# HSoumi/hybrid-als-twotower-recommender

Hardware: AMD Instinct MI355X
Metric: ALS epochs/sec + scored user-item pairs/sec at rank=64, 1/2/4/8 MI355X (higher is better)
Workload: dtype f64

## Files before the change

hybrid-als-twotower-recommender_amd/csrc/als_row.h:

```cpp
#pragma once
#include <type_traits>

#include "common.h"

#ifndef HREC_ALS_WAVES
#define HREC_ALS_WAVES 2
#endif
#ifndef HREC_ALS_CH0
#define HREC_ALS_CH0 8
#endif
#ifndef HREC_ALS_ABLATE
#define HREC_ALS_ABLATE 0
#endif
#ifndef HREC_ALS_SOLVE_UNROLL
#define HREC_ALS_SOLVE_UNROLL 8
#endif
#ifndef HREC_ALS_CH1
#define HREC_ALS_CH1 4
#endif
#ifndef HREC_ALS_PF
#define HREC_ALS_PF 8
#endif
#ifndef HREC_ALS_PF64
#define HREC_ALS_PF64 4
#endif
#ifndef HREC_ALS_ROT1DPP
#define HREC_ALS_ROT1DPP 1
#endif
#ifndef HREC_ALS_ROT1DPP64
#define HREC_ALS_ROT1DPP64 0
#endif
#ifndef HREC_ALS_PR
#define HREC_ALS_PR 2
#endif
#ifndef HREC_ALS_POOL_PF
#define HREC_ALS_POOL_PF 8
#endif
#ifndef HREC_ALS_POOL_PF64
#define HREC_ALS_POOL_PF64 4
#endif
#ifndef HREC_ALS_POOL_ROT1DPP64
#define HREC_ALS_POOL_ROT1DPP64 1
#endif

namespace hrec {

typedef double d4 __attribute__((ext_vector_type(4)));
typedef hrec_f4 f4;

template <int NT>
struct Vec;
template <>
struct Vec<4> {
  float x[4];
  __device__ static Vec load(const float* p) {
    const float4 t = *reinterpret_cast<const float4*>(p);
    return Vec{{t.x, t.y, t.z, t.w}};
  }
};
template <>
struct Vec<2> {
  float x[2];
  __device__ static Vec load(const float* p) {
    const float2 t = *reinterpret_cast<const float2*>(p);
    return Vec{{t.x, t.y}};
  }
};
template <>
struct Vec<1> {
  float x[1];
  __device__ static Vec load(const float* p) { return Vec{{*p}}; }
};

__device__ __forceinline__ int tri(int i) { return (i * (i + 1)) >> 1; }

typedef hrec_rsrc_t i4v;
typedef hrec_f2 f2;

struct VecD {
  double x[4];
};
__device__ __forceinline__ VecD struct_load_d(i4v rsrc, int vindex, int voffset) {
  const f4 lo = sbuf_load_f4(rsrc, vindex, voffset, 0, 0);
  const f4 hi = sbuf_load_f4(rsrc, vindex, voffset + 16, 0, 0);
  VecD v;
  v.x[0] = __hiloint2double(__float_as_int(lo.y), __float_as_int(lo.x));
  v.x[1] = __hiloint2double(__float_as_int(lo.w), __float_as_int(lo.z));
  v.x[2] = __hiloint2double(__float_as_int(hi.y), __float_as_int(hi.x));
  v.x[3] = __hiloint2double(__float_as_int(hi.w), __float_as_int(hi.z));
  return v;
}

struct VecD2 {
  double x[2];
};
__device__ __forceinline__ VecD2 struct_load_d2(i4v rsrc, int vindex, int voffset) {
  const f4 t = sbuf_load_f4(rsrc, vindex, voffset, 0, 0);
  VecD2 v;
  v.x[0] = __hiloint2double(__float_as_int(t.y), __float_as_int(t.x));
  v.x[1] = __hiloint2double(__float_as_int(t.w), __float_as_int(t.z));
  return v;
}

template <int NT>
__device__ __forceinline__ Vec<NT> struct_load(i4v rsrc, int vindex, int voffset) {
  Vec<NT> v;
  if constexpr (NT == 4) {
    const f4 t = sbuf_load_f4(rsrc, vindex, voffset, 0, 0);
    v.x[0] = t.x, v.x[1] = t.y, v.x[2] = t.z, v.x[3] = t.w;
  } else if constexpr (NT == 2) {
    const f2 t = sbuf_load_f2(rsrc, vindex, voffset, 0, 0);
    v.x[0] = t.x, v.x[1] = t.y;
  } else {
    v.x[0] = sbuf_load_f1(rsrc, vindex, voffset, 0, 0);
  }
  return v;
}

#ifdef HREC_ALS_STAMPS
__device__ unsigned long long g_als_stamps[8];
#define STAMP(i)                                                                      \
  do {                                                                                \
    __builtin_amdgcn_sched_barrier(0);                                                \
    const unsigned long long _t = __builtin_amdgcn_s_memtime();                       \
    __builtin_amdgcn_sched_barrier(0);                                                \
    if (threadIdx.x == 0 && (i) > 0) atomicAdd(&g_als_stamps[(i) > 0 ? (i) - 1 : 0], _t - _stamp_prev); \
    _stamp_prev = _t;                                                                 \
  } while (0)
#define STAMP_DECL unsigned long long _stamp_prev = 0
#else
#define STAMP(i) \
  do {           \
  } while (0)
#define STAMP_DECL
#endif

template <int N>
__device__ __forceinline__ double row_ror(double x) {
  const long long v = __double_as_longlong(x);
  const int lo = __builtin_amdgcn_mov_dpp((int)v, 0x120 + N, 0xf, 0xf, false);
  const int hi = __builtin_amdgcn_mov_dpp((int)(v >> 32), 0x120 + N, 0xf, 0xf, false);
  return __longlong_as_double(((long long)hi << 32) | (long long)(unsigned)lo);
}

__device__ __forceinline__ double bcast(double v, int src) {
  const long long x = __double_as_longlong(v);
  const int lo = __builtin_amdgcn_readlane((int)x, src);
  const int hi = __builtin_amdgcn_readlane((int)(x >> 32), src);
  return __longlong_as_double(((long long)hi << 32) | (long long)(unsigned)lo);
}

__device__ __forceinline__ void wave_lds_sync() {
  __builtin_amdgcn_fence(__ATOMIC_RELEASE, "wavefront");
  __builtin_amdgcn_wave_barrier();
  __builtin_amdgcn_fence(__ATOMIC_ACQUIRE, "wavefront");
}

template <int KP>
struct RowLds {
  static constexpr int kUp = KP * (KP + 1) / 2;
  static constexpr int kUpPad = ((kUp > 256 ? kUp : 256) + 1) & ~1;
  static constexpr int kSize = kUpPad + 128 + 3 * KP;
};

struct NoAcquire {};

template <int NT, int CH, int MODE, bool S64 = false, bool IMP = false, bool POOLED = false,
          typename Acq = NoAcquire>
__device__ __forceinline__ void gram_row(int64_t beg, int64_t end, int lane, const int32_t* __restrict__ indices,
                                         const float* __restrict__ values, const float* __restrict__ src,
                                         int64_t n_src, int k, double reg, d4 (&acc)[NT * (NT + 1) / 2],
                                         double* __restrict__ bsh, double* __restrict__ stage, double alpha = 0.0,
                                         const double* __restrict__ yty = nullptr, int* npos = nullptr,
                                         Acq acquire = Acq()) {
  constexpr bool kAcq = !std::is_same_v<Acq, NoAcquire>;
  static_assert(!kAcq || (NT == 4 && !IMP), "late slice acquisition: the kp-64 ring pipeline only");
  static_assert(!IMP || (MODE == 0 && !S64), "implicit feedback: f64 accumulation of f32 sources only");
  constexpr int KP = 16 * NT;
  constexpr int NPAIR = NT * (NT + 1) / 2;
  constexpr int CHN = 4 * CH;
  const int sub = lane >> 4;
  const int col = lane & 15;
  const int64_t n = end - beg;
  int n_pos = 0;

  STAMP_DECL;
  STAMP(0);
#pragma unroll
  for (int p = 0; p < NPAIR; ++p) acc[p] = d4{0.0, 0.0, 0.0, 0.0};
  if constexpr (HREC_ALS_ABLATE == 4) {
#pragma unroll
    for (int I = 0, p = 0; I < NT; p += NT - I, ++I)
#pragma unroll
      for (int rr = 0; rr < 4; ++rr) acc[p][rr] = (sub + 4 * rr == col) ? 1.0 + reg * (double)n : 0.0;
    if constexpr (kAcq) bsh = acquire() + RowLds<KP>::kUpPad + 128 + 2 * KP;
    if (lane < KP) bsh[lane] = 1.0;
    wave_lds_sync();
    return;
  }
  f4 fa[NPAIR];
  double bp[NT];
#pragma unroll
  for (int t = 0; t < NT; ++t) bp[t] = 0.0;

  auto load_iv = [&](int64_t base, int& ii, float& vv) {
    const int64_t p = base + (lane % CHN);
    const bool ok = (lane < CHN) && (p < end);
    ii = ok ? indices[p] : -1;
    vv = ok ? values[p] : 0.f;
  };
  auto gather = [&](Vec<NT> (&buf)[CH], int ii) {
#pragma unroll
    for (int s = 0; s < CH; ++s) {
      const int idx = __shfl(ii, 4 * s + sub, kWave);
      const int safe = idx < 0 ? 0 : idx;
      Vec<NT> v = Vec<NT>::load(src + (int64_t)safe * KP + NT * col);
#pragma unroll
      for (int t = 0; t < NT; ++t) v.x[t] = idx < 0 ? 0.f : v.x[t];
      buf[s] = v;
    }
  };

  if constexpr (NT == 4 && !IMP) {
  constexpr int PF = POOLED ? (S64 ? HREC_ALS_POOL_PF64 : HREC_ALS_POOL_PF) : (S64 ? HREC_ALS_PF64 : HREC_ALS_PF);
  static_assert(16 % PF == 0, "prefetch distance must divide the window");
  static_assert(!S64 || MODE == 0, "f64 sources: kp 64, f64 accumulation only");
  const int voff = (S64 ? 8 : 4) * NT * col;
  const int bp_addr = 4 * sub;
  const uint64_t sbase = (uint64_t)src;
  i4v rsrc;
  rsrc.x = __builtin_amdgcn_readfirstlane((int)(uint32_t)sbase);
  rsrc.y = __builtin_amdgcn_readfirstlane((int)(uint32_t)(sbase >> 32) | ((KP * (S64 ? 8 : 4)) << 16));
  rsrc.z = __builtin_amdgcn_readfirstlane((int)n_src);
  rsrc.w = 0x00020000;
  auto load_win = [&](int64_t w, int& ii, float& vv) {
    const int64_t p = beg + 64 * w + lane;
    const int64_t pc = p < end ? p : end - 1;
    const int iraw = indices[pc];
    const float vraw = values[pc];
    ii = p < end ? iraw : -1;
    vv = p < end ? vraw : 0.f;
  };
  auto bperm = [&](int win, int s) -> int { return __builtin_amdgcn_ds_bpermute(bp_addr + 16 * s, win); };
  const int64_t nsteps = (n + 3) >> 2;
  int iw0, iw1;
  float rw0, rw1;
  load_win(0, iw0, rw0);
  load_win(1, iw1, rw1);
  using RingT = std::conditional_t<S64, VecD, Vec<NT>>;
  auto ring_load = [&](int vi) -> RingT {
    if constexpr (S64) return struct_load_d(rsrc, vi, voff);
    else return struct_load<NT>(rsrc, vi, voff);
  };
  RingT ring[PF];
#pragma unroll
  for (int s = 0; s < PF; ++s) ring[s] = ring_load(bperm(iw0, s));
  int nidx = bperm(iw0, PF);
  constexpr bool kDiag4 = MODE == 0;
  constexpr int PR = HREC_ALS_PR;
  constexpr bool kRot1Dpp = S64 ? (POOLED ? HREC_ALS_POOL_ROT1DPP64 : HREC_ALS_ROT1DPP64) : HREC_ALS_ROT1DPP;
  static_assert(PR < PF, "rotated loads are issued from the current windows");
  const int voff1 = (S64 ? 8 : 4) * NT * ((col + 4) & 15), voff2 = (S64 ? 8 : 4) * NT * ((col + 8) & 15);
  auto rot_load = [&](int vi, int vo) -> RingT {
    if constexpr (S64) return struct_load_d(rsrc, vi, vo);
    else return struct_load<NT>(rsrc, vi, vo);
  };
  using PairT = std::conditional_t<S64, VecD2, Vec<2>>;
  const int hoff = (lane & 8) ? (S64 ? 16 : 8) : 0;
  auto pair_load = [&](int vi, int vo) -> PairT {
    if constexpr (S64) return struct_load_d2(rsrc, vi, vo);
    else return struct_load<2>(rsrc, vi, vo);
  };
  RingT rot1[PR];
  PairT rotA[PR], rotB[PR];
  if constexpr (kDiag4) {
#pragma unroll
    for (int q = 0; q < PR; ++q) {
      const int vi = bperm(iw0, q);
      if constexpr (!kRot1Dpp) rot1[q] = rot_load(vi, voff1);
      rotA[q] = pair_load(vi, voff + hoff);
      rotB[q] = pair_load(vi, voff2 + hoff);
    }
  }
  double dg[NT][3], dc[2];
#pragma unroll
  for (int t = 0; t < NT; ++t) dg[t][0] = dg[t][1] = 0.0;
#pragma unroll
  for (int t = 0; t < 2; ++t) dc[t] = 0.0;
  for (int64_t w = 0;; ++w) {
    int iw2;
    float rw2;
    load_win(w + 2, iw2, rw2);
    bool stop = false;
    const int rem = __builtin_amdgcn_readfirstlane((int)(nsteps - 16 * w < 16 ? nsteps - 16 * w : 16));
#pragma unroll
    for (int s = 0; s < 16; ++s) {
      if (s >= rem) {
        stop = true;
        break;
      }
      const RingT cur = ring[s % PF];
      double a[NT], ar1[NT], ar2[NT], apair[2];
#pragma unroll
      for (int t = 0; t < NT; ++t) a[t] = (double)cur.x[t];
      ring[s % PF] = ring_load(nidx);
      if constexpr (kDiag4) {
#pragma unroll
        for (int t = 0; t < NT; ++t) ar1[t] = kRot1Dpp ? row_ror<12>(a[t]) : (double)rot1[s % PR].x[t];
#pragma unroll
        for (int t = 0; t < 2; ++t) {
          apair[t] = (double)rotA[s % PR].x[t];
          ar2[t] = (double)rotB[s % PR].x[t];
        }
        const int vr = (s + PR < 16) ? bperm(iw0, s + PR) : bperm(iw1, s + PR - 16);
        if constexpr (!kRot1Dpp) rot1[s % PR] = rot_load(vr, voff1);
        rotA[s % PR] = pair_load(vr, voff + hoff);
        rotB[s % PR] = pair_load(vr, voff2 + hoff);
      }
      nidx = (s + 1 + PF < 16) ? bperm(iw0, s + 1 + PF) : bperm(iw1, s + 1 + PF - 16);
      const float rf = __int_as_float(__builtin_amdgcn_ds_bpermute(bp_addr + 16 * s, __float_as_int(rw0)));
      const double rv = (double)rf;
      if (MODE == 1 && (s % HREC_ALS_CH1) == 0) {
#pragma unroll
        for (int p = 0; p < NPAIR; ++p) fa[p] = f4{0.f, 0.f, 0.f, 0.f};
      }
      int p = 0;
#pragma unroll
      for (int I = 0; I < NT; ++I) {
#pragma unroll
        for (int J = I; J < NT; ++J) {
          if (MODE == 0) {
            if (I == J) {
              dg[I][0] = __builtin_amdgcn_mfma_f64_4x4x4f64(a[I], a[I], dg[I][0], 0, 0, 0);
              dg[I][1] = __builtin_amdgcn_mfma_f64_4x4x4f64(a[I], ar1[I], dg[I][1], 0, 0, 0);
              if (I < 2) dc[I] = __builtin_amdgcn_mfma_f64_4x4x4f64(apair[I], ar2[I], dc[I], 0, 0, 0);
            } else {
              acc[p] = __builtin_amdgcn_mfma_f64_16x16x4f64(a[I], a[J], acc[p], 0, 0, 0);
            }
          } else {
            fa[p] = __builtin_amdgcn_mfma_f32_16x16x4f32(cur.x[I], cur.x[J], fa[p], 0, 0, 0);
          }
          ++p;
        }
      }
#pragma unroll
      for (int t = 0; t < NT; ++t) bp[t] = fma(rv, a[t], bp[t]);
      if (MODE == 1 && ((s % HREC_ALS_CH1) == HREC_ALS_CH1 - 1 || s + 1 == rem)) {
#pragma unroll
        for (int p2 = 0; p2 < NPAIR; ++p2) {
#pragma unroll
          for (int rr = 0; rr < 4; ++rr) acc[p2][rr] += (double)fa[p2][rr];
        }
      }
    }
    if (stop || 16 * (w + 1) >= nsteps) break;
    iw0 = iw1;
    rw0 = rw1;
    iw1 = iw2;
    rw1 = rw2;
  }
  if constexpr (kAcq) {
    double* base = acquire();
    stage = base;
    bsh = base + RowLds<KP>::kUpPad + 128 + 2 * KP;
  }
  if constexpr (kDiag4) {
    const int i4 = lane >> 4, q4 = (lane >> 2) & 3, j4 = lane & 3;
#pragma unroll
    for (int I = 0, p = 0; I < NT; p += NT - I, ++I) {
#pragma unroll
      for (int sh = 0; sh < 3; ++sh) {
        const int r = 4 * q4 + i4, c = 4 * ((q4 + sh) & 3) + j4;
        if (sh == 2) {
          const bool mine = (q4 >= 2) == (I >= 2);
          const double v = dc[I & 1];
          stage[mine ? r * 16 + c : 256] = v;
          stage[mine ? c * 16 + r : 257] = v;
          continue;
        }
        stage[r * 16 + c] = dg[I][sh];
        stage[c * 16 + r] = dg[I][sh];
      }
      wave_lds_sync();
#pragma unroll
      for (int rr = 0; rr < 4; ++rr) acc[p][rr] = stage[(sub + 4 * rr) * 16 + col];
      wave_lds_sync();
    }
  }
  } else {
  int i0, i1;
  float r0, r1;
  load_iv(beg, i0, r0);
  load_iv(beg + CHN, i1, r1);
  Vec<NT> buf[CH];
  gather(buf, i0);

  for (int64_t base = beg; base < end; base += CHN) {
    Vec<NT> nbuf[CH];
    const bool more = base + CHN < end;
    if (more) gather(nbuf, i1);
    int i2;
    float r2;
    load_iv(base + 2 * CHN, i2, r2);
    if constexpr (IMP) n_pos += __builtin_popcountll(__ballot(r0 > 0.f));
    if (MODE == 1) {
#pragma unroll
      for (int p = 0; p < NPAIR; ++p) fa[p] = f4{0.f, 0.f, 0.f, 0.f};
    }
#pragma unroll
    for (int s = 0; s < CH; ++s) {
      const double rv = (double)__shfl(r0, 4 * s + sub, kWave);
      double a[NT];
#pragma unroll
      for (int t = 0; t < NT; ++t) a[t] = (double)buf[s].x[t];
      double aw[NT], bw = rv;
      if constexpr (IMP) {
        const double c1 = alpha * fabs(rv);
        bw = rv > 0.0 ? 1.0 + c1 : 0.0;
#pragma unroll
        for (int t = 0; t < NT; ++t) aw[t] = c1 * a[t];
      }
      auto lhs = [&](int t) -> double {
        if constexpr (IMP) return aw[t];
        else return a[t];
      };
      int p = 0;
#pragma unroll
      for (int I = 0; I < NT; ++I) {
#pragma unroll
        for (int J = I; J < NT; ++J) {
          if (MODE == 0)
            acc[p] = __builtin_amdgcn_mfma_f64_16x16x4f64(lhs(I), a[J], acc[p], 0, 0, 0);
          else
            fa[p] = __builtin_amdgcn_mfma_f32_16x16x4f32(buf[s].x[I], buf[s].x[J], fa[p], 0, 0, 0);
          ++p;
        }
      }
#pragma unroll
      for (int t = 0; t < NT; ++t) bp[t] = fma(bw, a[t], bp[t]);
    }
    if (MODE == 1) {
#pragma unroll
      for (int p = 0; p < NPAIR; ++p) {
#pragma unroll
        for (int rr = 0; rr < 4; ++rr) acc[p][rr] += (double)fa[p][rr];
      }
    }
    if (more) {
#pragma unroll
      for (int s = 0; s < CH; ++s) buf[s] = nbuf[s];
    }
    i0 = i1;
    r0 = r1;
    i1 = i2;
    r1 = r2;
  }
  }

  STAMP(1);
#pragma unroll
  for (int t = 0; t < NT; ++t) {
    bp[t] += __shfl_xor(bp[t], 16, kWave);
    bp[t] += __shfl_xor(bp[t], 32, kWave);
  }
  if (sub == 0) {
#pragma unroll
    for (int t = 0; t < NT; ++t) bsh[16 * t + col] = bp[t];
  }
  if (MODE == 1) {
#pragma unroll
    for (int p = 0; p < NPAIR; ++p) {
#pragma unroll
      for (int rr = 0; rr < 4; ++rr) stage[(4 * sub + rr) * 16 + col] = acc[p][rr];
      wave_lds_sync();
#pragma unroll
      for (int rr = 0; rr < 4; ++rr) acc[p][rr] = stage[(sub + 4 * rr) * 16 + col];
      wave_lds_sync();
    }
  }
  STAMP(2);
  if constexpr (IMP) {
    int p = 0;
#pragma unroll
    for (int I = 0; I < NT; ++I) {
#pragma unroll
      for (int J = I; J < NT; ++J) {
#pragma unroll
        for (int rr = 0; rr < 4; ++rr) acc[p][rr] += yty[(NT * (sub + 4 * rr) + I) * KP + NT * col + J];
        ++p;
      }
    }
    *npos = n_pos;
  }
  const double lambda = (double)(IMP ? (int64_t)n_pos : n) * reg;
  {
    int p = 0;
#pragma unroll
    for (int I = 0; I < NT; ++I) {
#pragma unroll
      for (int rr = 0; rr < 4; ++rr) {
        if (sub + 4 * rr == col) acc[p][rr] += (NT * col + I < k) ? lambda : 1.0;
      }
      p += NT - I;
    }
  }
}

template <int NT, bool LDSG>
__device__ __forceinline__ void factor_row_impl(int lane, d4 (&acc)[NT * (NT + 1) / 2], double* __restrict__ Up,
                                           double* __restrict__ scratch, const double* __restrict__ bsh,
                                           float* __restrict__ out) {
  constexpr int KP = 16 * NT;
  constexpr int NPAIR = NT * (NT + 1) / 2;
  double* __restrict__ colbuf = scratch;
  double* __restrict__ dsh = colbuf + 128;
  double* __restrict__ rdsh = dsh + KP;
  const int sub = lane >> 4, col = lane & 15;
  STAMP_DECL;
  STAMP(0);
  if constexpr (HREC_ALS_ABLATE == 1) {
    double sum = 0.0;
#pragma unroll
    for (int p = 0; p < NPAIR; ++p) sum += acc[p][0] + acc[p][1] + acc[p][2] + acc[p][3];
    wave_lds_sync();
    if (lane < KP) out[lane] = (float)(sum + bsh[lane]);
    return;
  }
  auto pidx = [](int I, int K) { return I * NT - (I * (I - 1)) / 2 + (K - I); };
  double bs = 0.0;
#pragma unroll
  for (int J = 0; J < NT; ++J) {
    if (!LDSG || J == 0) {
#pragma unroll
      for (int I = J; I < (LDSG ? NT : J + 1); ++I) {
#pragma unroll
        for (int K = I; K < NT; ++K) {
#pragma unroll
          for (int rr = 0; rr < 4; ++rr) {
            const int q = 16 * I + sub + 4 * rr, c = 16 * K + col;
            if (q <= c) Up[tri(c) + q] = acc[pidx(I, K)][rr];
          }
        }
      }
      wave_lds_sync();
    }
    if (J == 0) bs = lane < KP ? bsh[lane] : 0.0;
    const int c = lane;
    const bool own = c >= 16 * J && c < KP;
    double a[16];
#pragma unroll
    for (int m = 0; m < 16; ++m) {
      const int q = 16 * J + m;
      a[m] = (own && q <= c) ? Up[tri(c) + q] : 0.0;
    }
    double piv = bcast(a[0], 16 * J);
#pragma unroll
    for (int i = 0; i < 16; ++i) {
      const int pv = 16 * J + i;
      double* cb = colbuf + 64 * (i & 1);
      if (c < KP) cb[c] = a[i];
      const double r0 = __builtin_amdgcn_rcp(piv);
      const double r = fma(r0, fma(-piv, r0, 1.0), r0);
      const double ut = a[i] * r;
      if (own && c > pv) Up[tri(c) + pv] = ut;
      if (c == pv) {
        dsh[pv] = piv;
        rdsh[pv] = r;
      }
      {
        const double wq = bcast(bs, pv);
        if (own && c > pv) bs = fma(-ut, wq, bs);
      }
      if (i < 15) {
        piv = bcast(fma(-a[i], ut, a[i + 1]), pv + 1);
        wave_lds_sync();
#pragma unroll
        for (int m0 = (i + 1) & ~1; m0 < 16; m0 += 2) {
          const double2 u = *reinterpret_cast<const double2*>(cb + 16 * J + m0);
          if (m0 > i) a[m0] = fma(-u.x, ut, a[m0]);
          a[m0 + 1] = fma(-u.y, ut, a[m0 + 1]);
        }
      }
    }
    wave_lds_sync();
    if (J + 1 < NT) {
      double dq[4];
#pragma unroll
      for (int rr = 0; rr < 4; ++rr) dq[rr] = dsh[16 * J + sub + 4 * rr];
      d4 yv[NT];
#pragma unroll
      for (int K = J + 1; K < NT; ++K) {
#pragma unroll
        for (int rr = 0; rr < 4; ++rr) {
          const double x = Up[tri(16 * K + col) + 16 * J + sub + 4 * rr];
          acc[pidx(J, K)][rr] = x;
          yv[K][rr] = x * dq[rr];
        }
      }
#pragma unroll
      for (int K = J + 1; K < NT; ++K) {
#pragma unroll
        for (int M = K; M < NT; ++M) {
          if constexpr (LDSG) {
            d4 t;
#pragma unroll
            for (int rr = 0; rr < 4; ++rr) t[rr] = Up[tri(16 * M + col) + 16 * K + sub + 4 * rr];
#pragma unroll
            for (int rr = 0; rr < 4; ++rr)
              t = __builtin_amdgcn_mfma_f64_16x16x4f64(-acc[pidx(J, K)][rr], yv[M][rr], t, 0, 0, 0);
#pragma unroll
            for (int rr = 0; rr < 4; ++rr) {
              const int q = 16 * K + sub + 4 * rr, c = 16 * M + col;
              if (q <= c) Up[tri(c) + q] = t[rr];
            }
          } else {
#pragma unroll
            for (int rr = 0; rr < 4; ++rr)
              acc[pidx(K, M)] = __builtin_amdgcn_mfma_f64_16x16x4f64(-acc[pidx(J, K)][rr], yv[M][rr],
                                                                      acc[pidx(K, M)], 0, 0, 0);
          }
        }
      }
      if constexpr (LDSG) wave_lds_sync();
    }
  }
  STAMP(3);
  const int lc = lane < KP ? lane : KP - 1;
  const double myrd = rdsh[lc];
  if constexpr (HREC_ALS_ABLATE == 3) {
    if (lane < KP) out[lane] = (float)(myrd + Up[tri(lane)]);
    return;
  }
  double bi = bs * myrd;
#pragma unroll HREC_ALS_SOLVE_UNROLL
  for (int q = KP - 1; q >= 0; --q) {
    const double u = Up[tri(q) + (lane < KP ? lane : 0)];
    const double xq = bcast(bi, q);
    if (lane < q) bi = fma(-u, xq, bi);
  }
  STAMP(4);
  if (lane < KP) out[NT * (lane & 15) + (lane >> 4)] = (float)bi;
  wave_lds_sync();
}

template <int NT>
__device__ __forceinline__ void factor_row(int lane, d4 (&acc)[NT * (NT + 1) / 2], double* __restrict__ Up,
                                           double* __restrict__ scratch, const double* __restrict__ bsh,
                                           float* __restrict__ out) {
  factor_row_impl<NT, false>(lane, acc, Up, scratch, bsh, out);
}

template <int NT>
__device__ __forceinline__ void factor_row_lds(int lane, d4 (&acc)[NT * (NT + 1) / 2], double* __restrict__ Up,
                                               double* __restrict__ scratch, const double* __restrict__ bsh,
                                               float* __restrict__ out) {
  factor_row_impl<NT, true>(lane, acc, Up, scratch, bsh, out);
}

}
```

Measured before the change: 13.12.

## Block the in-panel Cholesky factorization into 4-column groups with MFMA trailing updates

Splits each 16-column panel factorization into groups of four columns. Scalar elimination runs only inside a group. The trailing update of the remaining sub-rows is done with f64 4x4x4 MFMA instructions on the accumulator registers, then written back to LDS. The goal is fewer per-lane scalar FMAs and smaller per-lane register arrays in the ALS normal-equation solve. In exchange it adds extra LDS round trips and barriers per group, and the accumulator layout now depends on MFMA semantics, which raises correctness risk.

```diff
diff --git a/hybrid-als-twotower-recommender_amd/csrc/als_row.h b/hybrid-als-twotower-recommender_amd/csrc/als_row.h
--- a/hybrid-als-twotower-recommender_amd/csrc/als_row.h
+++ b/hybrid-als-twotower-recommender_amd/csrc/als_row.h
@@ -512,6 +512,7 @@
                                            float* __restrict__ out) {
   constexpr int KP = 16 * NT;
   constexpr int NPAIR = NT * (NT + 1) / 2;
+  constexpr int G = 4;
   double* __restrict__ colbuf = scratch;
   double* __restrict__ dsh = colbuf + 128;
   double* __restrict__ rdsh = dsh + KP;
@@ -530,59 +531,91 @@
   double bs = 0.0;
 #pragma unroll
   for (int J = 0; J < NT; ++J) {
-    if (!LDSG || J == 0) {
-#pragma unroll
-      for (int I = J; I < (LDSG ? NT : J + 1); ++I) {
-#pragma unroll
-        for (int K = I; K < NT; ++K) {
-#pragma unroll
-          for (int rr = 0; rr < 4; ++rr) {
-            const int q = 16 * I + sub + 4 * rr, c = 16 * K + col;
-            if (q <= c) Up[tri(c) + q] = acc[pidx(I, K)][rr];
+    if constexpr (LDSG) {
+      if (J == 0) {
+#pragma unroll
+        for (int I = 0; I < NT; ++I) {
+#pragma unroll
+          for (int K = I; K < NT; ++K) {
+#pragma unroll
+            for (int rr = 0; rr < 4; ++rr) {
+              const int q = 16 * I + sub + 4 * rr, c = 16 * K + col;
+              if (q <= c) Up[tri(c) + q] = acc[pidx(I, K)][rr];
+            }
           }
         }
+        wave_lds_sync();
+      } else {
+#pragma unroll
+        for (int K = J; K < NT; ++K) {
+#pragma unroll
+          for (int rr = 1; rr < 4; ++rr) acc[pidx(J, K)][rr] = Up[tri(16 * K + col) + 16 * J + sub + 4 * rr];
+        }
+      }
+    } else {
+#pragma unroll
+      for (int K = J; K < NT; ++K) {
+        const int q = 16 * J + sub, c = 16 * K + col;
+        if (q <= c) Up[tri(c) + q] = acc[pidx(J, K)][0];
       }
       wave_lds_sync();
     }
     if (J == 0) bs = lane < KP ? bsh[lane] : 0.0;
     const int c = lane;
     const bool own = c >= 16 * J && c < KP;
-    double a[16];
-#pragma unroll
-    for (int m = 0; m < 16; ++m) {
-      const int q = 16 * J + m;
-      a[m] = (own && q <= c) ? Up[tri(c) + q] : 0.0;
-    }
-    double piv = bcast(a[0], 16 * J);
-#pragma unroll
-    for (int i = 0; i < 16; ++i) {
-      const int pv = 16 * J + i;
-      double* cb = colbuf + 64 * (i & 1);
-      if (c < KP) cb[c] = a[i];
-      const double r0 = __builtin_amdgcn_rcp(piv);
-      const double r = fma(r0, fma(-piv, r0, 1.0), r0);
-      const double ut = a[i] * r;
-      if (own && c > pv) Up[tri(c) + pv] = ut;
-      if (c == pv) {
-        dsh[pv] = piv;
-        rdsh[pv] = r;
-      }
-      {
-        const double wq = bcast(bs, pv);
-        if (own && c > pv) bs = fma(-ut, wq, bs);
-      }
-      if (i < 15) {
-        piv = bcast(fma(-a[i], ut, a[i + 1]), pv + 1);
+#pragma unroll
+    for (int g = 0; g < 16 / G; ++g) {
+      double a[G];
+#pragma unroll
+      for (int m = 0; m < G; ++m) {
+        const int q = 16 * J + G * g + m;
+        a[m] = (own && q <= c) ? Up[tri(c) + q] : 0.0;
+      }
+      double piv = bcast(a[0], 16 * J + G * g);
+#pragma unroll
+      for (int ii = 0; ii < G; ++ii) {
+        const int pv = 16 * J + G * g + ii;
+        double* cb = colbuf + 16 * ii;
+        if ((c >> 4) == J) cb[c & 15] = a[ii];
+        const double r0 = __builtin_amdgcn_rcp(piv);
+        const double r = fma(r0, fma(-piv, r0, 1.0), r0);
+        const double ut = a[ii] * r;
+        if (own && c > pv) Up[tri(c) + pv] = ut;
+        if (c == pv) {
+          dsh[pv] = piv;
+          rdsh[pv] = r;
+        }
+        {
+          const double wq = bcast(bs, pv);
+          if (own && c > pv) bs = fma(-ut, wq, bs);
+        }
+        if (ii < G - 1) {
+          piv = bcast(fma(-a[ii], ut, a[ii + 1]), pv + 1);
+          wave_lds_sync();
+#pragma unroll
+          for (int m = ii + 1; m < G; ++m) a[m] = fma(-cb[G * g + m], ut, a[m]);
+        }
+      }
+      wave_lds_sync();
+      if (g + 1 < 16 / G) {
+        double bu[NT];
+#pragma unroll
+        for (int K = J; K < NT; ++K) bu[K] = Up[tri(16 * K + col) + 16 * J + G * g + sub];
+#pragma unroll
+        for (int rr = g + 1; rr < 4; ++rr) {
+          const double am = -colbuf[16 * sub + 4 * rr + (col & 3)];
+#pragma unroll
+          for (int K = J; K < NT; ++K) {
+            acc[pidx(J, K)][rr] = __builtin_amdgcn_mfma_f64_4x4x4f64(am, bu[K], acc[pidx(J, K)][rr], 0, 0, 0);
+            if (rr == g + 1) {
+              const int q = 16 * J + sub + 4 * rr, cc = 16 * K + col;
+              if (q <= cc) Up[tri(cc) + q] = acc[pidx(J, K)][rr];
+            }
+          }
+        }
         wave_lds_sync();
-#pragma unroll
-        for (int m0 = (i + 1) & ~1; m0 < 16; m0 += 2) {
-          const double2 u = *reinterpret_cast<const double2*>(cb + 16 * J + m0);
-          if (m0 > i) a[m0] = fma(-u.x, ut, a[m0]);
-          a[m0 + 1] = fma(-u.y, ut, a[m0 + 1]);
-        }
-      }
-    }
-    wave_lds_sync();
+      }
+    }
     if (J + 1 < NT) {
       double dq[4];
 #pragma unroll
```

Result: no change. 13.20 (median of 6 runs) (+0.6%).
